# mistralai/mistral-inference

Measured on NVIDIA H100. Metric: decode tokens/sec (bf16, batch=1, seq=4k) [+ prefill TFLOPS, both vs roofline], higher is better.
Workload: dtype bf16

## Files before the change

### mistral_inference_b200/csrc/decode_megakernel.cuh

```cuda
#pragma once
#include "common.cuh"
#include "gemm_mma.cuh"

namespace mb200 {

constexpr int MK_CONSUMER_WARPS = 8;
constexpr int MK_CONSUMERS = MK_CONSUMER_WARPS * 32;
constexpr int MK_PRODUCER_WARPS = 2;
constexpr int MK_THREADS = MK_CONSUMERS + 32 * MK_PRODUCER_WARPS;
constexpr int MK_WEIGHT_STAGE_BYTES = 16 * 1024;
constexpr int MK_MAX_KC = MK_WEIGHT_STAGE_BYTES / 4;
constexpr int MK_KV_PAD = 16;
constexpr int MK_STAGE_BYTES = 16 * 1024 + 16 * MK_KV_PAD;
constexpr int MK_MAX_STAGES = 12;
constexpr int MK_MAX_SPLITS = 32;

struct MkLayer {
  const bf16* wqkv;
  const bf16* wo;
  const bf16* w13;
  const bf16* w2;
  const bf16* attn_norm;
  const bf16* ffn_norm;
  bf16* cache_k;
  bf16* cache_v;
};

struct MkParams {
  const MkLayer* layers;
  const int32_t* windows;
  int n_experts, top_k;
  const bf16* const* moe_gate;
  const bf16* const* moe_w13;
  const bf16* const* moe_w2;
  int n_layers;
  const bf16* emb;
  const bf16* final_norm;
  const bf16* w_out;
  const float* rope;
  const int64_t* token;
  int pos;
  int batch_row;
  float* logits;
  long long* next_token;
  unsigned long long* argmax_slots;
  int* argmax_counter;
  int dim, hidden, H, KV, vocab;
  float eps;
  int n_stages, xs_bytes;
  unsigned* bar_flags;
  unsigned* bar_epoch;
  int* done_counter;
  bf16* xbuf;
  bf16* hbuf;
  bf16* qbuf;
  bf16* abuf;
  bf16* gbuf;
  float* partial;
  unsigned long long* prof_bar;
  unsigned long long* prof;
};

__device__ __forceinline__ void mk_stamp(const MkParams& p, int tid, int layer, int idx) {
  if (p.prof != nullptr && tid == 0 && blockIdx.x % 21 == 0) {
    unsigned long long t;
    asm volatile("mov.u64 %0, %globaltimer;" : "=l"(t));
    p.prof[((blockIdx.x / 21) * p.n_layers + layer) * 16 + idx] = t;
  }
}

__device__ __forceinline__ uint32_t smem_u32(const void* p) { return (uint32_t)__cvta_generic_to_shared(p); }
__device__ __forceinline__ void mbar_init(uint64_t* bar, uint32_t count) {
  asm volatile("mbarrier.init.shared::cta.b64 [%0], %1;" ::"r"(smem_u32(bar)), "r"(count));
}
__device__ __forceinline__ void mbar_arrive(uint64_t* bar) {
  asm volatile("mbarrier.arrive.shared::cta.b64 _, [%0];" ::"r"(smem_u32(bar)) : "memory");
}
__device__ __forceinline__ void mbar_arrive_n(uint64_t* bar, uint32_t n) {
  asm volatile("mbarrier.arrive.shared::cta.b64 _, [%0], %1;" ::"r"(smem_u32(bar)), "r"(n) : "memory");
}
__device__ __forceinline__ void mbar_arrive_expect_tx(uint64_t* bar, uint32_t bytes) {
  asm volatile("mbarrier.arrive.expect_tx.shared::cta.b64 _, [%0], %1;" ::"r"(smem_u32(bar)), "r"(bytes) : "memory");
}
#ifndef MB200_WATCHDOG_SPINS
#define MB200_WATCHDOG_SPINS (1u << 22)
#endif
__device__ __forceinline__ bool mbar_try_wait(uint64_t* bar, uint32_t parity) {
  uint32_t ok;
  asm volatile(
      "{\n"
      ".reg .pred p;\n"
      "mbarrier.try_wait.parity.shared::cta.b64 p, [%1], %2;\n"
      "selp.u32 %0, 1, 0, p;\n"
      "}\n"
      : "=r"(ok)
      : "r"(smem_u32(bar)), "r"(parity)
      : "memory");
  return ok != 0;
}
__device__ __forceinline__ void mbar_wait(uint64_t* bar, uint32_t parity, int tag = 0, uint32_t it = 0) {
  uint32_t spins = 0;
  while (!mbar_try_wait(bar, parity)) {
    if (++spins == MB200_WATCHDOG_SPINS) {
      printf("[mb200 watchdog] block %d thread %d stuck in mbarrier wait tag=%d it=%u parity=%u\n", (int)blockIdx.x, (int)threadIdx.x, tag, it,
             parity);
      __trap();
    }
  }
}
__device__ __forceinline__ void mbar_wait_quiet(uint64_t* bar, uint32_t parity) {
  uint32_t spins = 0;
  while (!mbar_try_wait(bar, parity)) {
    if (++spins == MB200_WATCHDOG_SPINS) __trap();
  }
}
__device__ __forceinline__ void bulk_g2s(void* smem_dst, const void* gsrc, uint32_t bytes, uint64_t* bar) {
  asm volatile("cp.async.bulk.shared::cluster.global.mbarrier::complete_tx::bytes [%0], [%1], %2, [%3];" ::"r"(smem_u32(smem_dst)),
               "l"(gsrc), "r"(bytes), "r"(smem_u32(bar))
               : "memory");
}
__device__ __forceinline__ void consumer_sync() { asm volatile("bar.sync 1, %0;" ::"n"(MK_CONSUMERS) : "memory"); }

__device__ __forceinline__ uint4 ldcg16(const void* p) { return __ldcg(reinterpret_cast<const uint4*>(p)); }
__device__ __forceinline__ unsigned ld_acquire_u32(const unsigned* p) {
  unsigned v;
  asm volatile("ld.acquire.gpu.global.u32 %0, [%1];" : "=r"(v) : "l"(p) : "memory");
  return v;
}

constexpr int MK_BAR_WORDS = 8;
__device__ __forceinline__ void st_release_u32(unsigned* p, unsigned v) {
  asm volatile("st.release.gpu.global.u32 [%0], %1;" ::"l"(p), "r"(v) : "memory");
}
__device__ __forceinline__ void red_add_release_u32(unsigned* p, unsigned v) {
  asm volatile("red.release.gpu.global.add.u32 [%0], %1;" ::"l"(p), "r"(v) : "memory");
}
__device__ __forceinline__ void bar_stamp(const MkParams& p, int tid, int layer, int which, int leave) {
  if (p.prof_bar != nullptr && tid == 0) {
    unsigned long long t;
    asm volatile("mov.u64 %0, %globaltimer;" : "=l"(t));
    p.prof_bar[(((int64_t)blockIdx.x * p.n_layers + layer) * 6 + which) * 2 + leave] = t;
  }
}
__device__ __forceinline__ int bar_word_of(int cta) { return (cta * MK_BAR_WORDS) / (int)gridDim.x; }
__device__ __forceinline__ unsigned bar_word_count(int j) {
  const int G = (int)gridDim.x;
  const int lo = (j * G + MK_BAR_WORDS - 1) / MK_BAR_WORDS, hi = ((j + 1) * G + MK_BAR_WORDS - 1) / MK_BAR_WORDS;
  return (unsigned)(hi - lo);
}
__device__ __forceinline__ void grid_barrier(const MkParams& p, int tid, unsigned& epoch, int layer, int which) {
  ++epoch;
  bar_stamp(p, tid, layer, which, 0);
  consumer_sync();
  if (tid == 0) red_add_release_u32(p.bar_flags + bar_word_of(blockIdx.x) * 32, 1u);
  if (tid < MK_BAR_WORDS) {
    const unsigned target = epoch * bar_word_count(tid);
    unsigned spins = 0;
    while ((int)(ld_acquire_u32(p.bar_flags + tid * 32) - target) < 0) {
      if (++spins == MB200_WATCHDOG_SPINS) {
        printf("[mb200 watchdog] block %d stuck in grid barrier word %d target=%u counter=%u\n", (int)blockIdx.x, tid, target,
               ld_acquire_u32(p.bar_flags + tid * 32));
        __trap();
      }
    }
  }
  consumer_sync();
  bar_stamp(p, tid, layer, which, 1);
}

struct MatCut {
  int pairs, nch, kc, p0, p1;
};
__device__ __forceinline__ MatCut cut_matrix(int N, int K) {
  MatCut c;
  c.pairs = N >> 1;
  c.nch = (K + MK_MAX_KC - 1) / MK_MAX_KC;
  c.kc = K / c.nch;
  c.p0 = (int)(((long long)blockIdx.x * c.pairs) / gridDim.x);
  c.p1 = (int)(((long long)(blockIdx.x + 1) * c.pairs) / gridDim.x);
  return c;
}

constexpr int MK_MAX_TOPK = 4;
struct MoeRoute {
  int e[MK_MAX_TOPK];
  float w[MK_MAX_TOPK];
};

struct RingState {
  uint32_t it;
};


constexpr float kMaskedScore = -1.0e30f;

struct AttnSlice {
  int C, k_begin, k_end, n_kvst, pps, n_slices;
};
__device__ __forceinline__ AttnSlice attn_slice(const MkParams& p, int W) {
  AttnSlice a;
  const int len = min(p.pos + 1, W);
  a.C = (len + (int)gridDim.x - 1) / (int)gridDim.x;
  a.n_slices = (len + a.C - 1) / a.C;
  a.k_begin = min((int)blockIdx.x * a.C, len);
  a.k_end = min(a.k_begin + a.C, len);
  a.pps = min(16, (MK_STAGE_BYTES / (p.KV * kHeadDim * 2 + MK_KV_PAD)) & ~7);
  a.n_kvst = (a.k_end - a.k_begin + a.pps - 1) / a.pps;
  return a;
}

__device__ __forceinline__ void bulk_g2s_hint(void* smem_dst, const void* gsrc, uint32_t bytes, uint64_t* bar, uint64_t policy) {
  asm volatile("cp.async.bulk.shared::cluster.global.mbarrier::complete_tx::bytes.L2::cache_hint [%0], [%1], %2, [%3], %4;" ::"r"(
                   smem_u32(smem_dst)),
               "l"(gsrc), "r"(bytes), "r"(smem_u32(bar)), "l"(policy)
               : "memory");
}

constexpr int MK_INFLIGHT_CAP = 5;
static_assert(MK_INFLIGHT_CAP <= MK_CONSUMER_WARPS, "below the smallest ring decode_plan accepts (n_stages > MK_CONSUMER_WARPS)");

struct Producer {
  uint8_t* ring;
  uint64_t* full;
  uint64_t* empty;
  int n_stages;
  uint32_t it;
  uint64_t policy;
  int me;
  uint32_t slot, par;
  uint32_t cslot, cpar;

  __device__ __forceinline__ void advance() {
    ++it;
    if (++slot == (uint32_t)n_stages) {
      slot = 0;
      par ^= 1;
    }
    if (it > (uint32_t)MK_INFLIGHT_CAP && ++cslot == (uint32_t)n_stages) {
      cslot = 0;
      cpar ^= 1;
    }
  }
  __device__ __forceinline__ uint8_t* acquire(uint32_t bytes, uint64_t*& bar) {
    if ((int)(it % (uint32_t)MK_PRODUCER_WARPS) != me) {
      advance();
      return nullptr;
    }
    if (it >= (uint32_t)MK_INFLIGHT_CAP) mbar_wait(&full[cslot], cpar, 7, it);
    mbar_wait(&empty[slot], par ^ 1, 1, it);
    bar = &full[slot];
    mbar_arrive_expect_tx(bar, bytes);
    uint8_t* dst = ring + (size_t)slot * MK_STAGE_BYTES;
    advance();
    return dst;
  }

  __device__ __forceinline__ void pair_stage(const bf16* W, int K, const MatCut& c, int pair, int ch) {
    const uint32_t row_bytes = (uint32_t)c.kc * 2;
    const bf16* r0 = W + (int64_t)(2 * pair) * K;
    uint64_t* bar;
    uint8_t* dst = acquire(2 * row_bytes, bar);
    if (dst == nullptr) return;
    if (c.nch == 1) {
      bulk_g2s_hint(dst, r0, 2 * row_bytes, bar, policy);
    } else {
      bulk_g2s_hint(dst, r0 + ch * c.kc, row_bytes, bar, policy);
      bulk_g2s_hint(dst + row_bytes, r0 + K + ch * c.kc, row_bytes, bar, policy);
    }
  }

  __device__ __forceinline__ void matrix(const bf16* W, int N, int K) {
    const MatCut c = cut_matrix(N, K);
    for (int g0 = c.p0; g0 < c.p1; g0 += MK_CONSUMER_WARPS) {
      const int g = min(MK_CONSUMER_WARPS, c.p1 - g0);
      for (int ch = 0; ch < c.nch; ++ch)
        for (int w = 0; w < g; ++w) pair_stage(W, K, c, g0 + w, ch);
    }
  }

  __device__ __forceinline__ void moe_down(const bf16* const* w2, const int* sel, int top_k, int N, int K) {
    const MatCut c = cut_matrix(N, K);
    for (int g0 = c.p0; g0 < c.p1; g0 += MK_CONSUMER_WARPS) {
      const int g = min(MK_CONSUMER_WARPS, c.p1 - g0);
      for (int j = 0; j < top_k; ++j) {
        const bf16* W = w2[sel[j]];
        for (int ch = 0; ch < c.nch; ++ch)
          for (int w = 0; w < g; ++w) pair_stage(W, K, c, g0 + w, ch);
      }
    }
  }

  __device__ __forceinline__ void kv_slice(const MkParams& p, const MkLayer& L, int W) {
    const AttnSlice a = attn_slice(p, W);
    const int64_t row_elems = (int64_t)p.KV * kHeadDim;
    const uint32_t row_bytes = (uint32_t)row_elems * 2;
    const bf16* kbase = L.cache_k + ((int64_t)p.batch_row * W) * row_elems;
    const bf16* vbase = L.cache_v + ((int64_t)p.batch_row * W) * row_elems;
    for (int j = 0; j < a.n_kvst; ++j) {
      const int k0 = a.k_begin + j * a.pps;
      const int rows = min(a.pps, a.k_end - k0);
#pragma unroll
      for (int kv = 0; kv < 2; ++kv) {
        uint64_t* bar;
        uint8_t* dst = acquire((uint32_t)rows * row_bytes, bar);
        if (dst == nullptr) continue;
        const bf16* src = (kv ? vbase : kbase) + (int64_t)k0 * row_elems;
        for (int r = 0; r < rows; ++r) bulk_g2s_hint(dst + r * (row_bytes + MK_KV_PAD), src + (int64_t)r * row_elems, row_bytes, bar, policy);
      }
    }
  }
};

__device__ __forceinline__ void producer_main(const MkParams& p, uint8_t* ring, uint64_t* full, uint64_t* empty, int me, const MoeRoute* route,
                                              uint64_t* route_bar) {
  Producer pr;
  pr.ring = ring;
  pr.full = full;
  pr.empty = empty;
  pr.n_stages = p.n_stages;
  pr.it = 0;
  pr.me = me;
  pr.slot = pr.par = pr.cslot = pr.cpar = 0;
  asm volatile("createpolicy.fractional.L2::evict_first.b64 %0, 1.0;" : "=l"(pr.policy));
  const int q_dim = p.H * kHeadDim, kv_dim = p.KV * kHeadDim;
  for (int l = 0; l < p.n_layers; ++l) {
    const MkLayer L = p.layers[l];
    pr.matrix(L.wqkv, q_dim + 2 * kv_dim, p.dim);
    pr.kv_slice(p, L, p.windows[l]);
    pr.matrix(L.wo, p.dim, q_dim);
    if (p.n_experts == 0) {
      pr.matrix(L.w13, 2 * p.hidden, p.dim);
      pr.matrix(L.w2, p.dim, p.hidden);
    } else {
      mbar_wait(route_bar, (uint32_t)(l & 1), 8, (uint32_t)l);
      int sel[MK_MAX_TOPK];
      for (int j = 0; j < p.top_k; ++j) sel[j] = route->e[j];
      for (int j = 0; j < p.top_k; ++j) pr.matrix(p.moe_w13[l * p.n_experts + sel[j]], 2 * p.hidden, p.dim);
      pr.moe_down(p.moe_w2 + l * p.n_experts, sel, p.top_k, p.dim, p.hidden);
    }
  }
  pr.matrix(p.w_out, p.vocab, p.dim);
}

__device__ __forceinline__ void consume_pair_stage(const uint8_t* ring, uint64_t* full, uint64_t* empty, int n_stages, uint32_t it,
                                                   const uint4* xc, int kc8, int lane, float& a0, float& a1) {
  const uint32_t slot = it % n_stages, par = (it / n_stages) & 1;
  mbar_wait(&empty[slot], par ^ 1, 2, it);
  mbar_wait(&full[slot], par, 3, it);
  const uint4* w0 = reinterpret_cast<const uint4*>(ring + (size_t)slot * MK_STAGE_BYTES);
  const uint4* w1 = w0 + kc8;
#pragma unroll 4
  for (int i = lane; i < kc8; i += 32) {
    const uint4 a = w0[i], b = w1[i], x = xc[i];
    const uint32_t aw[4] = {a.x, a.y, a.z, a.w}, bw[4] = {b.x, b.y, b.z, b.w}, xw[4] = {x.x, x.y, x.z, x.w};
#pragma unroll
    for (int j = 0; j < 4; ++j) {
      const float xl = bf16lo(xw[j]), xh = bf16hi(xw[j]);
      a0 = fmaf(bf16lo(aw[j]), xl, a0);
      a0 = fmaf(bf16hi(aw[j]), xh, a0);
      a1 = fmaf(bf16lo(bw[j]), xl, a1);
      a1 = fmaf(bf16hi(bw[j]), xh, a1);
    }
  }
  __syncwarp();
  if (lane == 0) mbar_arrive_n(&empty[slot], MK_CONSUMER_WARPS);
}

template <class Pre, class Epi>
__device__ __forceinline__ void consume_matrix(int N, int K, const uint8_t* ring, uint64_t* full, uint64_t* empty, int n_stages, RingState& rs,
                                               const uint4* xs, int tid, Pre pre, Epi epi) {
  const MatCut c = cut_matrix(N, K);
  const int lane = tid & 31, warp = tid >> 5;
  const int kc8 = c.kc >> 3;
  for (int g0 = c.p0; g0 < c.p1; g0 += MK_CONSUMER_WARPS) {
    const int g = min(MK_CONSUMER_WARPS, c.p1 - g0);
    if (warp < g) {
      uint2 prefetched = make_uint2(0u, 0u);
      if (lane == 0) prefetched = pre(2 * (g0 + warp));
      float a0 = 0.f, a1 = 0.f;
      for (int ch = 0; ch < c.nch; ++ch)
        consume_pair_stage(ring, full, empty, n_stages, rs.it + (uint32_t)(ch * g + warp), xs + ch * kc8, kc8, lane, a0, a1);
      a0 = warp_sum(a0);
      a1 = warp_sum(a1);
      if (lane == 0) epi(2 * (g0 + warp), a0, a1, prefetched);
    }
    rs.it += (uint32_t)(g * c.nch);
    consumer_sync();
  }
}

__device__ __forceinline__ void stage_x(uint4* xs, const bf16* src, const bf16* norm_w, int K, float eps, float* red, int tid) {
  const int kc = K >> 3;
#pragma unroll 4
  for (int i = tid; i < kc; i += MK_CONSUMERS) xs[i] = ldcg16(reinterpret_cast<const uint4*>(src) + i);
  consumer_sync();
  if (norm_w == nullptr) return;
  const int lane = tid & 31, warp = tid >> 5;
  float ss = 0.f;
  for (int i = tid; i < kc; i += MK_CONSUMERS) {
    const uint4 v = xs[i];
    const uint32_t u[4] = {v.x, v.y, v.z, v.w};
#pragma unroll
    for (int j = 0; j < 4; ++j) {
      const float a = bf16lo(u[j]), b = bf16hi(u[j]);
      ss = fmaf(a, a, ss);
      ss = fmaf(b, b, ss);
    }
  }
  ss = warp_sum(ss);
  if (lane == 0) red[warp] = ss;
  consumer_sync();
  float tot = 0.f;
#pragma unroll
  for (int w = 0; w < MK_CONSUMER_WARPS; ++w) tot += red[w];
  const float r = ref_rsqrt(tot / (float)K + eps);
  const uint4* wn = reinterpret_cast<const uint4*>(norm_w);
  for (int i = tid; i < kc; i += MK_CONSUMERS) {
    const uint4 v = xs[i], g = wn[i];
    const uint32_t u[4] = {v.x, v.y, v.z, v.w}, gw[4] = {g.x, g.y, g.z, g.w};
    uint32_t o[4];
#pragma unroll
    for (int j = 0; j < 4; ++j)
      o[j] = pack_bf16x2(round_bf16(bf16lo(u[j]) * r) * bf16lo(gw[j]), round_bf16(bf16hi(u[j]) * r) * bf16hi(gw[j]));
    xs[i] = make_uint4(o[0], o[1], o[2], o[3]);
  }
  consumer_sync();
}

__device__ __forceinline__ uint32_t ldcg_u32(const void* p) { return __ldcg(reinterpret_cast<const unsigned int*>(p)); }

template <int REP, int PPS>
__device__ __forceinline__ void mk_attention_slice(const MkParams& p, const MkLayer& L, int W, uint8_t* ring, uint64_t* full, uint64_t* empty,
                                                   int n_stages, RingState& rs, int tid, int layer) {
  static_assert(REP <= 8, "query heads of a group are MMA rows 0..7");
  const AttnSlice a = attn_slice(p, W);
  if (a.n_kvst == 0) return;
  const int lane = tid & 31, warp = tid >> 5;
  const bool has_head = warp < p.KV;
  const int g = has_head ? warp : 0;
  const int row = lane >> 2, cq = lane & 3;
  const float sl2 = 0.08838834764831845f * kLog2e;
  const int64_t row_elems = (int64_t)p.KV * kHeadDim;
  const uint32_t row_stride = (uint32_t)row_elems * 2 + MK_KV_PAD;

  uint32_t qa[8][4];
#pragma unroll
  for (int ks = 0; ks < 8; ++ks) {
    qa[ks][0] = qa[ks][1] = qa[ks][2] = qa[ks][3] = 0u;
    if (row < REP) {
      const bf16* qp = p.qbuf + (g * REP + row) * kHeadDim + ks * 16 + cq * 2;
      qa[ks][0] = ldcg_u32(qp);
      qa[ks][2] = ldcg_u32(qp + 8);
    }
  }
  const int cur = p.pos % W;
  uint4 cur_kv = make_uint4(0, 0, 0, 0);
  if (cur >= a.k_begin && cur < a.k_end) {
    const bf16* base = (lane < 16 ? L.cache_k : L.cache_v);
    cur_kv = ldcg16(base + ((int64_t)p.batch_row * W + cur) * row_elems + (int64_t)g * kHeadDim + (lane & 15) * 8);
  }
  float o[16][4];
#pragma unroll
  for (int n = 0; n < 16; ++n) o[n][0] = o[n][1] = o[n][2] = o[n][3] = 0.f;
  float m_run = kMaskedScore, l_run = 0.f;

  for (int j = 0; j < a.n_kvst; ++j) {
    const uint32_t itk = rs.it + 2u * j, itv = itk + 1;
    const uint32_t sk = itk % n_stages, pk = (itk / n_stages) & 1, sv = itv % n_stages, pv = (itv / n_stages) & 1;
    mbar_wait(&full[sk], pk, 5, itk);
    mbar_wait(&full[sv], pv, 6, itv);
    if (j == 0) mk_stamp(p, tid, layer, 14);
    if (j == a.n_kvst - 1) mk_stamp(p, tid, layer, 15);
    if (has_head) {
      const int k0 = a.k_begin + j * PPS;
      const int nk = min(PPS, a.k_end - k0);
      uint8_t* kst = ring + (size_t)sk * MK_STAGE_BYTES + g * (kHeadDim * 2);
      uint8_t* vst = ring + (size_t)sv * MK_STAGE_BYTES + g * (kHeadDim * 2);
      if (cur >= k0 && cur < k0 + nk)
        *reinterpret_cast<uint4*>((lane < 16 ? kst : vst) + (size_t)(cur - k0) * row_stride + (lane & 15) * 16) = cur_kv;
      if (nk < PPS)
        for (int r = nk + (lane >> 4); r < PPS; r += 2) *reinterpret_cast<uint4*>(vst + (size_t)r * row_stride + (lane & 15) * 16) = make_uint4(0, 0, 0, 0);
      asm volatile("fence.proxy.async.shared::cta;" ::: "memory");
      __syncwarp();

      float sc[PPS / 8][4];
#pragma unroll
      for (int t = 0; t < PPS / 8; ++t) {
        sc[t][0] = sc[t][1] = sc[t][2] = sc[t][3] = 0.f;
        const uint32_t kaddr = smem_u32(kst) + (uint32_t)(t * 8 + (lane & 7)) * row_stride + (uint32_t)(lane >> 3) * 16;
#pragma unroll
        for (int k2 = 0; k2 < 4; ++k2) {
          uint32_t b0, b1, b2, b3;
          ldmatrix_x4(kaddr + k2 * 64, b0, b1, b2, b3);
          mma_bf16_16816(sc[t], qa[2 * k2], b0, b1);
          mma_bf16_16816(sc[t], qa[2 * k2 + 1], b2, b3);
        }
      }
      float mx = m_run;
#pragma unroll
      for (int t = 0; t < PPS / 8; ++t) {
#pragma unroll
        for (int c = 0; c < 2; ++c) {
          const int key = t * 8 + cq * 2 + c;
          sc[t][c] = key < nk ? sc[t][c] * sl2 : kMaskedScore;
          mx = fmaxf(mx, sc[t][c]);
        }
      }
      mx = fmaxf(mx, __shfl_xor_sync(0xffffffffu, mx, 1));
      mx = fmaxf(mx, __shfl_xor_sync(0xffffffffu, mx, 2));
      const float corr = exp2f(m_run - mx);
      m_run = mx;
      l_run *= corr;
      uint32_t pa[4] = {0u, 0u, 0u, 0u};
#pragma unroll
      for (int t = 0; t < PPS / 8; ++t) {
        const float e0 = exp2f(sc[t][0] - mx), e1 = exp2f(sc[t][1] - mx);
        l_run += e0 + e1;
        pa[2 * t] = pack_bf16x2(e0, e1);
      }
#pragma unroll
      for (int n = 0; n < 16; ++n) {
        o[n][0] *= corr;
        o[n][1] *= corr;
      }
      if constexpr (PPS == 16) {
        const uint32_t vaddr = smem_u32(vst) + (uint32_t)((lane & 7) + ((lane >> 3) & 1) * 8) * row_stride + (uint32_t)(lane >> 4) * 16;
#pragma unroll
        for (int n2 = 0; n2 < 8; ++n2) {
          uint32_t b0, b1, b2, b3;
          ldmatrix_x4_trans(vaddr + n2 * 32, b0, b1, b2, b3);
          mma_bf16_16816(o[2 * n2], pa, b0, b1);
          mma_bf16_16816(o[2 * n2 + 1], pa, b2, b3);
        }
      } else {
        const uint32_t vaddr = smem_u32(vst) + (uint32_t)(lane & 7) * row_stride + (uint32_t)(lane >> 3) * 16;
#pragma unroll
        for (int n4 = 0; n4 < 4; ++n4) {
          uint32_t b0, b1, b2, b3;
          ldmatrix_x4_trans(vaddr + n4 * 64, b0, b1, b2, b3);
          mma_bf16_16816(o[4 * n4], pa, b0, 0u);
          mma_bf16_16816(o[4 * n4 + 1], pa, b1, 0u);
          mma_bf16_16816(o[4 * n4 + 2], pa, b2, 0u);
          mma_bf16_16816(o[4 * n4 + 3], pa, b3, 0u);
        }
      }
    }
    __syncwarp();
    if (lane == 0) {
      mbar_arrive(&empty[sk]);
      mbar_arrive(&empty[sv]);
    }
  }
  rs.it += 2u * a.n_kvst;
  if (!has_head) return;
  l_run += __shfl_xor_sync(0xffffffffu, l_run, 1);
  l_run += __shfl_xor_sync(0xffffffffu, l_run, 2);
  if (row >= REP) return;
  m_run *= 0.6931471805599453f;
  const int PSTRIDE = kHeadDim + 2;
  float* mine = p.partial + ((int64_t)blockIdx.x * p.H + g * REP + row) * PSTRIDE;
#pragma unroll
  for (int n = 0; n < 16; ++n) *reinterpret_cast<float2*>(mine + 2 + n * 8 + cq * 2) = make_float2(o[n][0], o[n][1]);
  if (cq == 0) *reinterpret_cast<float2*>(mine) = make_float2(m_run, l_run);
}

constexpr int MK_CMB_MAX = 20;
__device__ __forceinline__ void mk_attention_combine(const MkParams& p, int W, int tid, float* scratch) {
  const AttnSlice a = attn_slice(p, W);
  const int lane = tid & 31, warp = tid >> 5;
  const int PSTRIDE = kHeadDim + 2;
  float* sm = scratch;
  for (int u = blockIdx.x; u < p.H * 4; u += gridDim.x) {
    const int h = u >> 2, q4 = u & 3;
    float m = kMaskedScore, l = 0.f, acc = 0.f;
    for (int a0 = warp; a0 < a.n_slices; a0 += MK_CONSUMER_WARPS * MK_CMB_MAX) {
      float mt[MK_CMB_MAX], lt[MK_CMB_MAX], at[MK_CMB_MAX];
#pragma unroll
      for (int i = 0; i < MK_CMB_MAX; ++i) {
        const int sl = a0 + i * MK_CONSUMER_WARPS;
        mt[i] = kMaskedScore;
        lt[i] = at[i] = 0.f;
        if (sl < a.n_slices) {
          const float* pp = p.partial + ((int64_t)sl * p.H + h) * PSTRIDE;
          const float2 ml = __ldcg(reinterpret_cast<const float2*>(pp));
          mt[i] = ml.x;
          lt[i] = ml.y;
          at[i] = __ldcg(pp + 2 + q4 * 32 + lane);
        }
      }
      float mn = m;
#pragma unroll
      for (int i = 0; i < MK_CMB_MAX; ++i) mn = fmaxf(mn, mt[i]);
      const float c0 = exp2f((m - mn) * kLog2e);
      l *= c0;
      acc *= c0;
#pragma unroll
      for (int i = 0; i < MK_CMB_MAX; ++i) {
        const float c1 = exp2f((mt[i] - mn) * kLog2e);
        l = fmaf(lt[i], c1, l);
        acc = fmaf(at[i], c1, acc);
      }
      m = mn;
    }
    sm[warp * 34 + 2 + lane] = acc;
    if (lane == 0) {
      sm[warp * 34] = m;
      sm[warp * 34 + 1] = l;
    }
    consumer_sync();
    if (warp == 0) {
      float mn = kMaskedScore;
#pragma unroll
      for (int w = 0; w < MK_CONSUMER_WARPS; ++w) mn = fmaxf(mn, sm[w * 34]);
      float lt = 0.f, at = 0.f;
#pragma unroll
      for (int w = 0; w < MK_CONSUMER_WARPS; ++w) {
        const float mw = sm[w * 34];
        const float c = exp2f((mw - mn) * kLog2e);
        lt += sm[w * 34 + 1] * c;
        at += sm[w * 34 + 2 + lane] * c;
      }
      p.abuf[h * kHeadDim + q4 * 32 + lane] = __float2bfloat16_rn(at / lt);
    }
    consumer_sync();
  }
}


__device__ __forceinline__ void moe_route(const MkParams& p, int layer, const uint4* xs, float* red, MoeRoute* route, uint64_t* route_bar, int tid) {
  const int lane = tid & 31, warp = tid >> 5;
  const bf16* gate = p.moe_gate[layer];
  const int kc = p.dim >> 3;
  for (int e = warp; e < p.n_experts; e += MK_CONSUMER_WARPS) {
    const uint4* wrow = reinterpret_cast<const uint4*>(gate + (int64_t)e * p.dim);
    float acc = 0.f;
    for (int i = lane; i < kc; i += 32) {
      const uint4 a = __ldg(wrow + i), x = xs[i];
      const uint32_t aw[4] = {a.x, a.y, a.z, a.w}, xw[4] = {x.x, x.y, x.z, x.w};
#pragma unroll
      for (int j = 0; j < 4; ++j) {
        acc = fmaf(bf16lo(aw[j]), bf16lo(xw[j]), acc);
        acc = fmaf(bf16hi(aw[j]), bf16hi(xw[j]), acc);
      }
    }
    acc = warp_sum(acc);
    if (lane == 0) red[8 + e] = round_bf16(acc);
  }
  consumer_sync();
  if (tid == 0) {
    int sel[MK_MAX_TOPK];
    float val[MK_MAX_TOPK];
    unsigned taken = 0;
    for (int j = 0; j < p.top_k; ++j) {
      int best = -1;
      for (int e = 0; e < p.n_experts; ++e)
        if (!((taken >> e) & 1u) && (best < 0 || red[8 + e] > red[8 + best])) best = e;
      taken |= 1u << best;
      sel[j] = best;
      val[j] = red[8 + best];
    }
    float den = 0.f, ex[MK_MAX_TOPK];
    for (int j = 0; j < p.top_k; ++j) {
      ex[j] = expf(val[j] - val[0]);
      den += ex[j];
    }
    for (int j = 0; j < p.top_k; ++j) val[j] = round_bf16(ex[j] / den);
    for (int a = 1; a < p.top_k; ++a)
      for (int b = a; b > 0 && sel[b] < sel[b - 1]; --b) {
        const int ts = sel[b];
        sel[b] = sel[b - 1];
        sel[b - 1] = ts;
        const float tv = val[b];
        val[b] = val[b - 1];
        val[b - 1] = tv;
      }
    for (int j = 0; j < p.top_k; ++j) {
      route->e[j] = sel[j];
      route->w[j] = val[j];
    }
    mbar_arrive(route_bar);
  }
  consumer_sync();
}

template <class Pre, class Epi>
__device__ __forceinline__ void consume_moe_down(const MkParams& p, const MoeRoute& rt, const uint8_t* ring, uint64_t* full, uint64_t* empty,
                                                 int n_stages, RingState& rs, const uint4* xs, int tid, Pre pre, Epi epi) {
  const MatCut c = cut_matrix(p.dim, p.hidden);
  const int lane = tid & 31, warp = tid >> 5;
  const int kc8 = c.kc >> 3;
  const int hid8 = p.hidden >> 3;
  for (int g0 = c.p0; g0 < c.p1; g0 += MK_CONSUMER_WARPS) {
    const int g = min(MK_CONSUMER_WARPS, c.p1 - g0);
    if (warp < g) {
      uint2 prefetched = make_uint2(0u, 0u);
      if (lane == 0) prefetched = pre(2 * (g0 + warp));
      float r0 = 0.f, r1 = 0.f;
      for (int j = 0; j < p.top_k; ++j) {
        float a0 = 0.f, a1 = 0.f;
        for (int ch = 0; ch < c.nch; ++ch)
          consume_pair_stage(ring, full, empty, n_stages, rs.it + (uint32_t)((j * c.nch + ch) * g + warp), xs + j * hid8 + ch * kc8, kc8,
                             lane, a0, a1);
        a0 = warp_sum(a0);
        a1 = warp_sum(a1);
        const float t0 = round_bf16(rt.w[j] * round_bf16(a0)), t1 = round_bf16(rt.w[j] * round_bf16(a1));
        r0 = (j == 0) ? t0 : round_bf16(r0 + t0);
        r1 = (j == 0) ? t1 : round_bf16(r1 + t1);
      }
      if (lane == 0) epi(2 * (g0 + warp), r0, r1, prefetched);
    }
    rs.it += (uint32_t)(g * c.nch * p.top_k);
    consumer_sync();
  }
}

template <int REP>
__global__ void __launch_bounds__(MK_THREADS, 1) decode_megakernel(const MkParams p) {
  extern __shared__ __align__(128) uint8_t smem[];
  uint8_t* ring = smem;
  uint4* xs = reinterpret_cast<uint4*>(smem + (size_t)p.n_stages * MK_STAGE_BYTES);
  uint64_t* full = reinterpret_cast<uint64_t*>(reinterpret_cast<uint8_t*>(xs) + p.xs_bytes);
  uint64_t* empty = full + MK_MAX_STAGES;
  float* red = reinterpret_cast<float*>(empty + MK_MAX_STAGES);
  MoeRoute* route = reinterpret_cast<MoeRoute*>(red + 48);
  uint64_t* route_bar = reinterpret_cast<uint64_t*>(route + 1);

  const int tid = threadIdx.x;
  if (tid == 0) {
    for (int i = 0; i < p.n_stages; ++i) {
      mbar_init(&full[i], 1);
      mbar_init(&empty[i], MK_CONSUMER_WARPS);
    }
    mbar_init(route_bar, 1);
    asm volatile("fence.mbarrier_init.release.cluster;" ::: "memory");
  }
  __syncthreads();

  const int q_dim = p.H * kHeadDim, kv_dim = p.KV * kHeadDim;
  RingState rs;
  rs.it = 0;

  if (tid >= MK_CONSUMERS) {
    if ((tid & 31) == 0) producer_main(p, ring, full, empty, (tid - MK_CONSUMERS) >> 5, route, route_bar);
    return;
  }

  unsigned epoch = ld_acquire_u32(p.bar_epoch);
  const int64_t token = *p.token;
  for (int l = 0; l < p.n_layers; ++l) {
    const MkLayer L = p.layers[l];
    const int W = p.windows[l];
    const bf16* x_in = (l == 0) ? p.emb + token * p.dim : p.xbuf + (size_t)(l & 1) * p.dim;
    bf16* x_out = p.xbuf + (size_t)((l + 1) & 1) * p.dim;

    mk_stamp(p, tid, l, 0);
    stage_x(xs, x_in, L.attn_norm, p.dim, p.eps, red, tid);
    mk_stamp(p, tid, l, 1);
    {
      const int slot_row = p.batch_row * W + p.pos % W;
      const float* rope_row = p.rope + (int64_t)p.pos * (kHeadDim / 2) * 2;
      bf16* ck = L.cache_k + (int64_t)slot_row * kv_dim;
      bf16* cv = L.cache_v + (int64_t)slot_row * kv_dim;
      consume_matrix(q_dim + 2 * kv_dim, p.dim, ring, full, empty, p.n_stages, rs, xs, tid,
                     [&](int n) { return *reinterpret_cast<const uint2*>(rope_row + ((n & (kHeadDim - 1)) >> 1) * 2); },
                     [&](int n, float a0, float a1, uint2 pf) {
        const float y0 = round_bf16(a0), y1 = round_bf16(a1);
        if (n < q_dim + kv_dim) {
          const float2 cs = make_float2(__uint_as_float(pf.x), __uint_as_float(pf.y));
          float re, im;
          ref_cmul(y0, y1, cs.x, cs.y, re, im);
          const uint32_t packed = pack_bf16x2(re, im);
          if (n < q_dim)
            *reinterpret_cast<uint32_t*>(p.qbuf + n) = packed;
          else
            *reinterpret_cast<uint32_t*>(ck + (n - q_dim)) = packed;
        } else {
          *reinterpret_cast<uint32_t*>(cv + (n - q_dim - kv_dim)) = pack_bf16x2(y0, y1);
        }
      });
    }
    mk_stamp(p, tid, l, 2);
    grid_barrier(p, tid, epoch, l, 0);
    mk_stamp(p, tid, l, 3);

    if (attn_slice(p, W).pps == 16)
      mk_attention_slice<REP, 16>(p, L, W, ring, full, empty, p.n_stages, rs, tid, l);
    else
      mk_attention_slice<REP, 8>(p, L, W, ring, full, empty, p.n_stages, rs, tid, l);
    mk_stamp(p, tid, l, 12);
    grid_barrier(p, tid, epoch, l, 1);
    mk_stamp(p, tid, l, 13);
    mk_attention_combine(p, W, tid, reinterpret_cast<float*>(xs));
    mk_stamp(p, tid, l, 4);
    grid_barrier(p, tid, epoch, l, 2);
    mk_stamp(p, tid, l, 5);

    stage_x(xs, p.abuf, nullptr, q_dim, 0.f, red, tid);
    consume_matrix(p.dim, q_dim, ring, full, empty, p.n_stages, rs, xs, tid, [&](int n) { return make_uint2(ldcg_u32(x_in + n), 0u); }, [&](int n, float a0, float a1, uint2 pf) {
      const uint32_t r = pf.x;
      *reinterpret_cast<uint32_t*>(p.hbuf + n) = pack_bf16x2(round_bf16(a0) + bf16lo(r), round_bf16(a1) + bf16hi(r));
    });
    mk_stamp(p, tid, l, 6);
    grid_barrier(p, tid, epoch, l, 3);
    mk_stamp(p, tid, l, 7);

    if (p.n_experts == 0) {
      stage_x(xs, p.hbuf, L.ffn_norm, p.dim, p.eps, red, tid);
      consume_matrix(2 * p.hidden, p.dim, ring, full, empty, p.n_stages, rs, xs, tid, [&](int) { return make_uint2(0u, 0u); }, [&](int n, float a0, float a1, uint2) {
        const float s = round_bf16(ref_silu(round_bf16(a0)));
        p.gbuf[n >> 1] = __float2bfloat16_rn(s * round_bf16(a1));
      });
      mk_stamp(p, tid, l, 8);
      grid_barrier(p, tid, epoch, l, 4);
      mk_stamp(p, tid, l, 9);

      stage_x(xs, p.gbuf, nullptr, p.hidden, 0.f, red, tid);
      consume_matrix(p.dim, p.hidden, ring, full, empty, p.n_stages, rs, xs, tid, [&](int n) { return make_uint2(ldcg_u32(p.hbuf + n), 0u); },
                     [&](int n, float a0, float a1, uint2 pf) {
                       const uint32_t r = pf.x;
                       *reinterpret_cast<uint32_t*>(x_out + n) = pack_bf16x2(round_bf16(a0) + bf16lo(r), round_bf16(a1) + bf16hi(r));
                     });
    } else {
      stage_x(xs, p.hbuf, L.ffn_norm, p.dim, p.eps, red, tid);
      moe_route(p, l, xs, red, route, route_bar, tid);
      const MoeRoute rt = *route;
      for (int j = 0; j < p.top_k; ++j) {
        bf16* gj = p.gbuf + (size_t)j * p.hidden;
        consume_matrix(2 * p.hidden, p.dim, ring, full, empty, p.n_stages, rs, xs, tid, [&](int) { return make_uint2(0u, 0u); },
                       [&](int n, float a0, float a1, uint2) {
                         const float sv = round_bf16(ref_silu(round_bf16(a0)));
                         gj[n >> 1] = __float2bfloat16_rn(sv * round_bf16(a1));
                       });
      }
      mk_stamp(p, tid, l, 8);
      grid_barrier(p, tid, epoch, l, 4);
      mk_stamp(p, tid, l, 9);
      stage_x(xs, p.gbuf, nullptr, p.top_k * p.hidden, 0.f, red, tid);
      consume_moe_down(p, rt, ring, full, empty, p.n_stages, rs, xs, tid, [&](int n) { return make_uint2(ldcg_u32(p.hbuf + n), 0u); },
                       [&](int n, float r0, float r1, uint2 pf) {
                         *reinterpret_cast<uint32_t*>(x_out + n) = pack_bf16x2(r0 + bf16lo(pf.x), r1 + bf16hi(pf.x));
                       });
    }
    mk_stamp(p, tid, l, 10);
    grid_barrier(p, tid, epoch, l, 5);
    mk_stamp(p, tid, l, 11);
  }

  stage_x(xs, p.xbuf + (size_t)(p.n_layers & 1) * p.dim, p.final_norm, p.dim, p.eps, red, tid);
  unsigned long long best = 0ull;
  auto key_of = [](float v, int idx) {
    unsigned u = __float_as_uint(v);
    u = (u & 0x80000000u) ? ~u : (u | 0x80000000u);
    return ((unsigned long long)u << 32) | (unsigned)(0x7fffffff - idx);
  };
  consume_matrix(p.vocab, p.dim, ring, full, empty, p.n_stages, rs, xs, tid, [&](int) { return make_uint2(0u, 0u); },
                 [&](int n, float a0, float a1, uint2) {
                   const float y0 = round_bf16(a0), y1 = round_bf16(a1);
                   *reinterpret_cast<float2*>(p.logits + n) = make_float2(y0, y1);
                   const unsigned long long k0 = key_of(y0, n), k1 = key_of(y1, n + 1);
                   best = max(best, max(k0, k1));
                 });
  if (p.next_token != nullptr) {
    unsigned long long* sm_best = reinterpret_cast<unsigned long long*>(xs);
    consumer_sync();
    if ((tid & 31) == 0) sm_best[tid >> 5] = best;
    consumer_sync();
    if (tid == 0) {
      unsigned long long b = 0ull;
#pragma unroll
      for (int w = 0; w < MK_CONSUMER_WARPS; ++w) b = max(b, sm_best[w]);
      p.argmax_slots[blockIdx.x] = b;
      __threadfence();
      const int prev = atomicAdd(p.argmax_counter, 1);
      if (prev == (int)gridDim.x - 1) {
        *p.argmax_counter = 0;
        __threadfence();
        unsigned long long g = 0ull;
        for (int c = 0; c < (int)gridDim.x; ++c) g = max(g, __ldcg(p.argmax_slots + c));
        *p.next_token = (long long)(0x7fffffff - (int)(g & 0xffffffffull));
      }
    }
  }
  consumer_sync();
  if (tid == 0) {
    __threadfence();
    const int prev = atomicAdd(p.done_counter, 1);
    if (prev == (int)gridDim.x - 1) {
      *p.done_counter = 0;
      st_release_u32(p.bar_epoch, epoch);
    }
  }
}

}
```

Baseline: 175.0.

## Flatten producer loops into a resumable walk state machine with stall profiling

Replaces the producer's nested per-matrix, per-KV and per-expert loops with a flat Walk iterator that yields one stage copy per step and packs the MoE routing selection into a 32-bit word. The wait on the full and empty barriers becomes a combined try-wait spin with a watchdog, and optional per-layer profiling counters record producer stall times in widened profiling rows. The intent looks like simpler producer control flow and instrumentation of producer stalls. The extra index arithmetic per stage (divisions in stage()) could add producer latency.

```diff
diff --git a/mistral_inference_b200/csrc/decode_megakernel.cuh b/mistral_inference_b200/csrc/decode_megakernel.cuh
--- a/mistral_inference_b200/csrc/decode_megakernel.cuh
+++ b/mistral_inference_b200/csrc/decode_megakernel.cuh
@@ -61,11 +61,14 @@
   unsigned long long* prof;
 };
 
+constexpr int MK_PROF_STAMPS = 16;
+constexpr int MK_PROF_WORDS = 24;
+constexpr unsigned long long MK_PROF_LONG_NS = 1000;
 __device__ __forceinline__ void mk_stamp(const MkParams& p, int tid, int layer, int idx) {
   if (p.prof != nullptr && tid == 0 && blockIdx.x % 21 == 0) {
     unsigned long long t;
     asm volatile("mov.u64 %0, %globaltimer;" : "=l"(t));
-    p.prof[((blockIdx.x / 21) * p.n_layers + layer) * 16 + idx] = t;
+    p.prof[((blockIdx.x / 21) * p.n_layers + layer) * MK_PROF_WORDS + idx] = t;
   }
 }
 
@@ -209,12 +212,137 @@
   return a;
 }
 
+struct StageCopy {
+  const bf16* src;
+  int64_t src_step;
+  uint32_t bytes, dst_step;
+  int count;
+};
+
+enum : int { SEG_QKV, SEG_KV, SEG_WO, SEG_UP, SEG_DOWN };
+
+struct Walk {
+  uint32_t it;
+  int layer, seg, e, s, n;
+  MatCut c;
+  int k_begin, k_end, pps;
+  const bf16* W;
+  const bf16* V;
+
+  __device__ __forceinline__ bool done(const MkParams& p) const { return layer > p.n_layers; }
+  __device__ __forceinline__ bool gated(const MkParams& p, int routed) const {
+    return p.n_experts != 0 && layer < p.n_layers && seg == SEG_UP && e == 0 && routed != layer;
+  }
+  __device__ __forceinline__ void matrix(const bf16* w, int N, int K) {
+    W = w;
+    c = cut_matrix(N, K);
+    n = (c.p1 - c.p0) * c.nch;
+  }
+  __device__ __forceinline__ int experts(const MkParams& p) const { return (seg == SEG_DOWN && p.n_experts) ? p.top_k : 1; }
+  __device__ __forceinline__ void setup(const MkParams& p, uint32_t sel) {
+    const int q_dim = p.H * kHeadDim, kv_dim = p.KV * kHeadDim;
+    s = 0;
+    if (layer == p.n_layers) {
+      matrix(p.w_out, p.vocab, p.dim);
+      return;
+    }
+    const MkLayer& L = p.layers[layer];
+    if (seg == SEG_QKV) {
+      matrix(L.wqkv, q_dim + 2 * kv_dim, p.dim);
+    } else if (seg == SEG_KV) {
+      const int win = p.windows[layer];
+      const AttnSlice a = attn_slice(p, win);
+      k_begin = a.k_begin;
+      k_end = a.k_end;
+      pps = a.pps;
+      n = 2 * a.n_kvst;
+      W = L.cache_k + ((int64_t)p.batch_row * win) * kv_dim;
+      V = L.cache_v + ((int64_t)p.batch_row * win) * kv_dim;
+    } else if (seg == SEG_WO) {
+      matrix(L.wo, p.dim, q_dim);
+    } else if (seg == SEG_UP) {
+      matrix(p.n_experts ? p.moe_w13[layer * p.n_experts + ((sel >> (8 * e)) & 0xff)] : L.w13, 2 * p.hidden, p.dim);
+    } else {
+      matrix(L.w2, p.dim, p.hidden);
+      n *= experts(p);
+    }
+  }
+  __device__ __forceinline__ void next_segment(const MkParams& p) {
+    if (layer == p.n_layers) {
+      ++layer;
+      return;
+    }
+    if (seg == SEG_UP && ++e < (p.n_experts ? p.top_k : 1)) return;
+    e = 0;
+    if (++seg > SEG_DOWN) {
+      seg = SEG_QKV;
+      ++layer;
+    }
+  }
+  __device__ __forceinline__ void settle(const MkParams& p, uint32_t sel, int routed) {
+    for (;;) {
+      n = 0;
+      if (done(p) || gated(p, routed)) return;
+      setup(p, sel);
+      if (n > 0) return;
+      next_segment(p);
+    }
+  }
+  __device__ __forceinline__ void next(const MkParams& p, uint32_t sel, int routed) {
+    ++it;
+    if (++s < n) return;
+    next_segment(p);
+    settle(p, sel, routed);
+  }
+
+  __device__ __forceinline__ StageCopy stage(const MkParams& p, uint32_t sel) const {
+    StageCopy sc;
+    if (seg == SEG_KV) {
+      const int64_t row_elems = (int64_t)p.KV * kHeadDim;
+      const int k0 = k_begin + (s >> 1) * pps;
+      sc.src = ((s & 1) ? V : W) + (int64_t)k0 * row_elems;
+      sc.src_step = row_elems;
+      sc.bytes = (uint32_t)row_elems * 2;
+      sc.dst_step = sc.bytes + MK_KV_PAD;
+      sc.count = min(pps, k_end - k0);
+      return sc;
+    }
+    const int ne = experts(p), K = c.kc * c.nch;
+    const int per_group = MK_CONSUMER_WARPS * c.nch * ne;
+    const int gi = s / per_group, r = s - gi * per_group;
+    const int g0 = c.p0 + gi * MK_CONSUMER_WARPS, g = min(MK_CONSUMER_WARPS, c.p1 - g0);
+    const int j = r / (c.nch * g), r2 = r - j * (c.nch * g);
+    const int ch = r2 / g, w = r2 - ch * g;
+    const bf16* m = (seg == SEG_DOWN && p.n_experts) ? p.moe_w2[layer * p.n_experts + ((sel >> (8 * j)) & 0xff)] : W;
+    const bf16* r0 = m + (int64_t)(2 * (g0 + w)) * K;
+    sc.bytes = (uint32_t)c.kc * 2;
+    if (c.nch == 1) {
+      sc.src = r0;
+      sc.src_step = 0;
+      sc.bytes *= 2;
+      sc.dst_step = 0;
+      sc.count = 1;
+    } else {
+      sc.src = r0 + ch * c.kc;
+      sc.src_step = K;
+      sc.dst_step = sc.bytes;
+      sc.count = 2;
+    }
+    return sc;
+  }
+};
+
 __device__ __forceinline__ void bulk_g2s_hint(void* smem_dst, const void* gsrc, uint32_t bytes, uint64_t* bar, uint64_t policy) {
   asm volatile("cp.async.bulk.shared::cluster.global.mbarrier::complete_tx::bytes.L2::cache_hint [%0], [%1], %2, [%3], %4;" ::"r"(
                    smem_u32(smem_dst)),
                "l"(gsrc), "r"(bytes), "r"(smem_u32(bar)), "l"(policy)
                : "memory");
 }
+__device__ __forceinline__ unsigned long long globaltimer() {
+  unsigned long long t;
+  asm volatile("mov.u64 %0, %globaltimer;" : "=l"(t));
+  return t;
+}
 
 constexpr int MK_INFLIGHT_CAP = 5;
 static_assert(MK_INFLIGHT_CAP <= MK_CONSUMER_WARPS, "below the smallest ring decode_plan accepts (n_stages > MK_CONSUMER_WARPS)");
@@ -224,90 +352,52 @@
   uint64_t* full;
   uint64_t* empty;
   int n_stages;
-  uint32_t it;
   uint64_t policy;
   int me;
   uint32_t slot, par;
   uint32_t cslot, cpar;
-
-  __device__ __forceinline__ void advance() {
-    ++it;
+  uint32_t sel;
+  int routed;
+  unsigned long long* prof;
+
+  __device__ __forceinline__ bool owns(uint32_t it) const { return (int)(it % (uint32_t)MK_PRODUCER_WARPS) == me; }
+  __device__ __forceinline__ void advance(uint32_t it) {
     if (++slot == (uint32_t)n_stages) {
       slot = 0;
       par ^= 1;
     }
-    if (it > (uint32_t)MK_INFLIGHT_CAP && ++cslot == (uint32_t)n_stages) {
+    if (it + 1 > (uint32_t)MK_INFLIGHT_CAP && ++cslot == (uint32_t)n_stages) {
       cslot = 0;
       cpar ^= 1;
     }
   }
-  __device__ __forceinline__ uint8_t* acquire(uint32_t bytes, uint64_t*& bar) {
-    if ((int)(it % (uint32_t)MK_PRODUCER_WARPS) != me) {
-      advance();
-      return nullptr;
-    }
-    if (it >= (uint32_t)MK_INFLIGHT_CAP) mbar_wait(&full[cslot], cpar, 7, it);
-    mbar_wait(&empty[slot], par ^ 1, 1, it);
-    bar = &full[slot];
-    mbar_arrive_expect_tx(bar, bytes);
+
+  __device__ __forceinline__ void copy(const MkParams& p, const Walk& cp) {
+    bool landed = cp.it < (uint32_t)MK_INFLIGHT_CAP || mbar_try_wait(&full[cslot], cpar);
+    if (!landed || !mbar_try_wait(&empty[slot], par ^ 1)) {
+      const unsigned long long t0 = prof != nullptr ? globaltimer() : 0ull;
+      unsigned long long t_landed = t0;
+      for (uint32_t spins = 0;;) {
+        if (!landed && mbar_try_wait(&full[cslot], cpar)) {
+          landed = true;
+          if (prof != nullptr) t_landed = globaltimer();
+        }
+        if (landed && mbar_try_wait(&empty[slot], par ^ 1)) break;
+        if (++spins == MB200_WATCHDOG_SPINS) __trap();
+      }
+      if (prof != nullptr) {
+        const unsigned long long full_ns = globaltimer() - t_landed;
+        unsigned long long* row = prof + (int64_t)min(cp.layer, p.n_layers - 1) * MK_PROF_WORDS + MK_PROF_STAMPS;
+        row[me] += full_ns;
+        row[2 + me] += t_landed - t0;
+        if (full_ns >= MK_PROF_LONG_NS) row[4 + me] += full_ns;
+      }
+    }
+    const StageCopy sc = cp.stage(p, sel);
+    uint64_t* bar = &full[slot];
+    mbar_arrive_expect_tx(bar, sc.bytes * (uint32_t)sc.count);
     uint8_t* dst = ring + (size_t)slot * MK_STAGE_BYTES;
-    advance();
-    return dst;
-  }
-
-  __device__ __forceinline__ void pair_stage(const bf16* W, int K, const MatCut& c, int pair, int ch) {
-    const uint32_t row_bytes = (uint32_t)c.kc * 2;
-    const bf16* r0 = W + (int64_t)(2 * pair) * K;
-    uint64_t* bar;
-    uint8_t* dst = acquire(2 * row_bytes, bar);
-    if (dst == nullptr) return;
-    if (c.nch == 1) {
-      bulk_g2s_hint(dst, r0, 2 * row_bytes, bar, policy);
-    } else {
-      bulk_g2s_hint(dst, r0 + ch * c.kc, row_bytes, bar, policy);
-      bulk_g2s_hint(dst + row_bytes, r0 + K + ch * c.kc, row_bytes, bar, policy);
-    }
-  }
-
-  __device__ __forceinline__ void matrix(const bf16* W, int N, int K) {
-    const MatCut c = cut_matrix(N, K);
-    for (int g0 = c.p0; g0 < c.p1; g0 += MK_CONSUMER_WARPS) {
-      const int g = min(MK_CONSUMER_WARPS, c.p1 - g0);
-      for (int ch = 0; ch < c.nch; ++ch)
-        for (int w = 0; w < g; ++w) pair_stage(W, K, c, g0 + w, ch);
-    }
-  }
-
-  __device__ __forceinline__ void moe_down(const bf16* const* w2, const int* sel, int top_k, int N, int K) {
-    const MatCut c = cut_matrix(N, K);
-    for (int g0 = c.p0; g0 < c.p1; g0 += MK_CONSUMER_WARPS) {
-      const int g = min(MK_CONSUMER_WARPS, c.p1 - g0);
-      for (int j = 0; j < top_k; ++j) {
-        const bf16* W = w2[sel[j]];
-        for (int ch = 0; ch < c.nch; ++ch)
-          for (int w = 0; w < g; ++w) pair_stage(W, K, c, g0 + w, ch);
-      }
-    }
-  }
-
-  __device__ __forceinline__ void kv_slice(const MkParams& p, const MkLayer& L, int W) {
-    const AttnSlice a = attn_slice(p, W);
-    const int64_t row_elems = (int64_t)p.KV * kHeadDim;
-    const uint32_t row_bytes = (uint32_t)row_elems * 2;
-    const bf16* kbase = L.cache_k + ((int64_t)p.batch_row * W) * row_elems;
-    const bf16* vbase = L.cache_v + ((int64_t)p.batch_row * W) * row_elems;
-    for (int j = 0; j < a.n_kvst; ++j) {
-      const int k0 = a.k_begin + j * a.pps;
-      const int rows = min(a.pps, a.k_end - k0);
-#pragma unroll
-      for (int kv = 0; kv < 2; ++kv) {
-        uint64_t* bar;
-        uint8_t* dst = acquire((uint32_t)rows * row_bytes, bar);
-        if (dst == nullptr) continue;
-        const bf16* src = (kv ? vbase : kbase) + (int64_t)k0 * row_elems;
-        for (int r = 0; r < rows; ++r) bulk_g2s_hint(dst + r * (row_bytes + MK_KV_PAD), src + (int64_t)r * row_elems, row_bytes, bar, policy);
-      }
-    }
+    for (int r = 0; r < sc.count; ++r) bulk_g2s_hint(dst + r * sc.dst_step, sc.src + r * sc.src_step, sc.bytes, bar, policy);
   }
 };
 
@@ -318,28 +408,30 @@
   pr.full = full;
   pr.empty = empty;
   pr.n_stages = p.n_stages;
-  pr.it = 0;
   pr.me = me;
   pr.slot = pr.par = pr.cslot = pr.cpar = 0;
+  pr.sel = 0;
+  pr.routed = -1;
+  pr.prof = (p.prof != nullptr && blockIdx.x % 21 == 0) ? p.prof + (int64_t)(blockIdx.x / 21) * p.n_layers * MK_PROF_WORDS : nullptr;
   asm volatile("createpolicy.fractional.L2::evict_first.b64 %0, 1.0;" : "=l"(pr.policy));
-  const int q_dim = p.H * kHeadDim, kv_dim = p.KV * kHeadDim;
-  for (int l = 0; l < p.n_layers; ++l) {
-    const MkLayer L = p.layers[l];
-    pr.matrix(L.wqkv, q_dim + 2 * kv_dim, p.dim);
-    pr.kv_slice(p, L, p.windows[l]);
-    pr.matrix(L.wo, p.dim, q_dim);
-    if (p.n_experts == 0) {
-      pr.matrix(L.w13, 2 * p.hidden, p.dim);
-      pr.matrix(L.w2, p.dim, p.hidden);
-    } else {
-      mbar_wait(route_bar, (uint32_t)(l & 1), 8, (uint32_t)l);
-      int sel[MK_MAX_TOPK];
-      for (int j = 0; j < p.top_k; ++j) sel[j] = route->e[j];
-      for (int j = 0; j < p.top_k; ++j) pr.matrix(p.moe_w13[l * p.n_experts + sel[j]], 2 * p.hidden, p.dim);
-      pr.moe_down(p.moe_w2 + l * p.n_experts, sel, p.top_k, p.dim, p.hidden);
-    }
-  }
-  pr.matrix(p.w_out, p.vocab, p.dim);
+  Walk cp;
+  cp.it = 0;
+  cp.layer = cp.seg = cp.e = 0;
+  cp.settle(p, pr.sel, pr.routed);
+  while (!cp.done(p)) {
+    if (cp.n == 0) {
+      mbar_wait(route_bar, (uint32_t)(cp.layer & 1), 8, (uint32_t)cp.layer);
+      uint32_t sel = 0;
+      for (int j = 0; j < p.top_k; ++j) sel |= (uint32_t)route->e[j] << (8 * j);
+      pr.sel = sel;
+      pr.routed = cp.layer;
+      cp.settle(p, pr.sel, pr.routed);
+      continue;
+    }
+    if (pr.owns(cp.it)) pr.copy(p, cp);
+    pr.advance(cp.it);
+    cp.next(p, pr.sel, pr.routed);
+  }
 }
 
 __device__ __forceinline__ void consume_pair_stage(const uint8_t* ring, uint64_t* full, uint64_t* empty, int n_stages, uint32_t it,
```

After: 180.6 (median of 6 runs). +3.2%, better.
